# yhwu/rsicnv

Measured on AMD Instinct MI355X. Metric: bases/sec through RSI pipeline (bin+GC+NB+segment), higher is better.
Workload: dtype int32

## Files before the change

### include/rsi_hot.h

```cpp
#ifndef RSI_HOT_H
#define RSI_HOT_H
#include <stdint.h>
#ifdef __cplusplus
extern "C" {
#endif

typedef enum rsi_status {
  RSI_OK = 0,
  RSI_ERR_NO_DEVICE = -1,
  RSI_ERR_BAD_ARG = -2,
  RSI_ERR_HIP = -3,
  RSI_ERR_TOO_SMALL = -4,
  RSI_ERR_UNSUPPORTED = -5,
  RSI_ERR_INTERNAL = -6
} rsi_status;

typedef struct rsi_params {
  int32_t m;
  int32_t gcadjust;
  int32_t trans;
  int32_t merge;
  int32_t maxchkbp;
  int32_t debug;
  double cap;
// ... 165 lines not shown

int rsi_result_ncalls(const rsi_result* r, int which);
const rsi_call* rsi_result_calls(const rsi_result* r, int which);
const rsi_chrom_stats* rsi_result_stats(const rsi_result* r);
int rsi_result_noncode(const rsi_result* r, int32_t* pairs, int cap);
int rsi_result_format_row(const rsi_result* r, int i, const char* chrom, char* buf, int cap);
void rsi_result_free(rsi_result* r);

int64_t rsi_hot_fetch_i32(rsi_ctx* ctx, const char* name, int32_t* out, int64_t cap);
int64_t rsi_hot_fetch_f32(rsi_ctx* ctx, const char* name, float* out, int64_t cap);
int64_t rsi_hot_fetch_i64(rsi_ctx* ctx, const char* name, int64_t* out, int64_t cap);

int rsi_hot_debug_level_sums(rsi_ctx* ctx, const float* T, const int32_t* status, int64_t nb, int Lmax, float* sums, int32_t* counts);
int rsi_hot_debug_scan(rsi_ctx* ctx, const float* T, const int32_t* medint, int64_t nb, double RDmedian, double tmedian, double tlamda,
                       int Lmax, int32_t* status, int32_t* info);
int rsi_hot_debug_grid_median(rsi_ctx* ctx, const float* x, const int32_t* mask, int64_t nb, int mode, double center, double* out,
                              int32_t* info);
int rsi_hot_debug_grid_mad_i32(rsi_ctx* ctx, const int32_t* x, int64_t nb, double center, double* out, int32_t* info);

int rsi_hot_debug_classify(rsi_ctx* ctx, const uint8_t* fasta, int64_t n, const int64_t* start, const int64_t* end, int count,
                           uint64_t* gcbits, uint64_t* nbits);

int rsi_hot_debug_per_base(rsi_ctx* ctx, const rsi_params* p, const int32_t* depth, const uint8_t* fasta, int64_t n, const int64_t* start,
                           const int64_t* end, int count, rsi_chrom_stats* out);

int rsi_hot_kernel_times(const rsi_ctx* ctx, const char** names, float* ms, int cap);
int rsi_hot_phase_times(const rsi_ctx* ctx, const char** names, double* ms, int cap);
void rsi_hot_set_timing(rsi_ctx* ctx, int on);
void rsi_hot_set_timing_kernel(rsi_ctx* ctx, const char* name);

// ... 44 lines not shown
```

### rsicnv_amd/api.py

```python
import contextlib
import ctypes as C
import os

import numpy as np

POOL_HW_QUEUES, MIN_HW_QUEUES = 32, 4


def _queue_count(s):
    return int(s) if s is not None and 1 <= len(s) <= 9 and all(c in "0123456789" for c in s) else -1


def _process_setup(env=os.environ):
    user = env.get("RSI_HOT_HW_QUEUES")
    if user != "keep":
        want = _queue_count(user)
        if want >= 0:
            env["GPU_MAX_HW_QUEUES"] = str(min(POOL_HW_QUEUES, max(MIN_HW_QUEUES, want)))
        elif _queue_count(env.get("GPU_MAX_HW_QUEUES")) < POOL_HW_QUEUES:
            env["GPU_MAX_HW_QUEUES"] = str(POOL_HW_QUEUES)
    return max(0, _queue_count(env.get("GPU_MAX_HW_QUEUES")))


HW_QUEUES = _process_setup()

_HERE = os.path.dirname(os.path.abspath(__file__))
LIB_PATH = os.environ.get("RSI_HOT_LIB") or os.path.join(_HERE, "librsi_hot.so")

RSI_OK = 0
STATUS_NAMES = {0: "RSI_OK", -1: "RSI_ERR_NO_DEVICE", -2: "RSI_ERR_BAD_ARG", -3: "RSI_ERR_HIP",
                -4: "RSI_ERR_TOO_SMALL", -5: "RSI_ERR_UNSUPPORTED", -6: "RSI_ERR_INTERNAL"}

EXPORTS = ["rsi_default_params", "rsi_hot_create", "rsi_hot_destroy", "rsi_hot_last_error", "rsi_hot_run",
           "rsi_hot_run_device", "rsi_hot_load_depth_text", "rsi_hot_run_text", "rsi_hot_load_depth_bam", "rsi_hot_run_bam", "rsi_bam_references", "rsi_result_annotate_bam", "rsi_result_summary", "rsi_summary_format_row", "rsi_summary_format_rows", "rsi_result_pairs", "rsi_result_ncalls", "rsi_result_calls", "rsi_result_stats", "rsi_result_noncode",
           "rsi_result_format_row", "rsi_result_free", "rsi_hot_fetch_i32", "rsi_hot_fetch_f32", "rsi_hot_fetch_i64",
           "rsi_hot_kernel_times", "rsi_hot_phase_times", "rsi_hot_set_timing", "rsi_hot_process_setup", "rsi_pool_create", "rsi_pool_destroy", "rsi_pool_workers", "rsi_pool_hw_queues", "rsi_pool_worker",
           "rsi_pool_set_timing", "rsi_pool_set_timing_kernel", "rsi_hot_set_timing_kernel", "rsi_pool_set_schedule", "rsi_pool_last_error", "rsi_pool_run", "rsi_pool_run_host", "rsi_pool_submit", "rsi_pool_wait", "rsi_plot_expand", "rsi_plot_write_files", "rsi_result_log_line", "rsi_hot_debug_level_sums", "rsi_hot_debug_scan", "rsi_hot_debug_grid_median", "rsi_hot_debug_grid_mad_i32", "rsi_synth_generate_host", "rsi_synth_generate_device", "rsi_synth_write_depth_text", "rsi_synth_write_fasta", "rsi_synth_append_genome_text",
           "rsi_genome_text_open", "rsi_genome_text_next", "rsi_genome_text_release", "rsi_genome_text_copy_depth",
           "rsi_genome_text_kernel_ms", "rsi_genome_text_close", "rsi_genome_text_last_error", "rsi_hot_run_depth_device",
           "rsi_hot_last_inflate_stats", "rsi_hot_inflate_bgzf", "rsi_genome_text_inflate_stats",
           "rsi_synth_append_genome_bgzf", "rsi_genome_text_open_samples", "rsi_genome_text_samples", "rsi_genome_text_max_resident",
           "rsi_genome_text_sample_depth", "rsi_genome_text_copy_sample_depth", "rsi_synth_append_genome_samples",
           "rsi_genome_bedgraph_open", "rsi_synth_append_genome_bedgraph", "rsi_genome_bedgraph_open_indexed", "rsi_genome_text_index_range",
           "rsi_hot_set_exclude", "rsi_exclude_read_bed", "rsi_hot_debug_classify", "rsi_hot_debug_per_base",
           "rsi_hot_write_track", "rsi_hot_write_track_device", "rsi_hot_debug_track",
           "rsi_hot_write_bin_track", "rsi_hot_debug_bin_track",
           "rsi_hot_set_track_format", "rsi_hot_last_deflate_stats", "rsi_bgzf_write_eof", "rsi_hot_debug_deflate",
           "rsi_track_index_create", "rsi_track_index_free", "rsi_hot_set_track_index", "rsi_track_index_append",
           "rsi_track_index_write_tbi", "rsi_track_index_counts", "rsi_track_index_debug_tbi"]


class RsiParams(C.Structure):
# ... 401 lines not shown
        self._check(self.lib.rsi_hot_debug_level_sums(self.ctx, t.ctypes.data, s.ctypes.data, t.size, int(Lmax), sums.ctypes.data, counts.ctypes.data))
        return sums, counts

    def debug_scan(self, T, medint, RDmedian, tmedian, tlamda, Lmax):
        t = np.ascontiguousarray(T, dtype=np.float32)
        mi = np.ascontiguousarray(medint, dtype=np.int32)
        assert t.size == mi.size
        st = np.zeros(t.size, dtype=np.int32)
        info = np.zeros(4, dtype=np.int32)
        self.lib.rsi_hot_debug_scan.argtypes = [C.c_void_p, C.c_void_p, C.c_void_p, C.c_int64, C.c_double, C.c_double, C.c_double, C.c_int,
                                                C.c_void_p, C.c_void_p]
        self._check(self.lib.rsi_hot_debug_scan(self.ctx, t.ctypes.data, mi.ctypes.data, t.size, float(RDmedian), float(tmedian), float(tlamda),
                                                int(Lmax), st.ctypes.data, info.ctypes.data))
        return st, info

    GRID_MODES = {"pair": 0, "mad": 1, "host": 2}

    def debug_grid_median(self, x, mask=None, mode="pair", center=0.0):
        out = np.zeros(4, dtype=np.float64)
        info = np.zeros(8, dtype=np.int32)
        if mode == "med":
            assert mask is None
            xi = np.ascontiguousarray(x, dtype=np.int32)
            self.lib.rsi_hot_debug_grid_mad_i32.argtypes = [C.c_void_p, C.c_void_p, C.c_int64, C.c_double, C.c_void_p, C.c_void_p]
            self._check(self.lib.rsi_hot_debug_grid_mad_i32(self.ctx, xi.ctypes.data, xi.size, float(center), out.ctypes.data, info.ctypes.data))
            return out, info
        xf = np.ascontiguousarray(x, dtype=np.float32)
        mk = None if mask is None else np.ascontiguousarray(mask, dtype=np.int32)
        assert mk is None or mk.size == xf.size
        self.lib.rsi_hot_debug_grid_median.argtypes = [C.c_void_p, C.c_void_p, C.c_void_p, C.c_int64, C.c_int, C.c_double, C.c_void_p, C.c_void_p]
# ... 506 lines not shown
```

### rsicnv_amd/csrc/hostmath.h

```cpp
#pragma once
#include <math.h>
#include <stddef.h>
#include <stdint.h>
#include <algorithm>
#include <vector>

namespace rsih {

struct Quantiles { double lqt, med, uqt; };

template <class T>
inline double grid_step(const T*) { return 0.01; }
template <>
inline double grid_step<int>(const int*) { return 1.0; }

void bucket_indices_f32(const float* x, size_t n, double lo, double dy, uint32_t* idx);

template <class T>
Quantiles grid_quantiles(const T* x, size_t n) {
  const double dy = grid_step(x);
  double lo = x[0], hi = x[0], acc = 0;
  for (size_t i = 0; i < n; ++i) {
    acc += x[i];
    if (x[i] < lo) lo = x[i];
// ... 98 lines not shown
  }
  return med;
}

template <class T>
double variance_pop(const T* y, size_t n) {
  double s1 = 0.0, s2 = 0.0;
  for (size_t i = 0; i < n; ++i) { s1 += (double)y[i]; s2 += (double)y[i] * (double)y[i]; }
  const double mu = s1 / double(n);
  return s2 / double(n) - mu * mu;
}

double normal_cdf(double x);

template <class Pred>
double last_true(Pred pred) {
  if (!pred(0.0)) return -1.0;
  union { double d; uint64_t u; } lo, hi, mid;
  lo.d = 0.0; hi.d = INFINITY;
  if (pred(hi.d)) return INFINITY;
  while (hi.u - lo.u > 1) {
    mid.u = lo.u + (hi.u - lo.u) / 2;
    if (pred(mid.d)) lo = mid; else hi = mid;
  }
  return lo.d;
}
template <class Pred>
double first_true(Pred pred) {
  if (pred(0.0)) return 0.0;
  union { double d; uint64_t u; } lo, hi, mid;
  lo.d = 0.0; hi.d = INFINITY;
  if (!pred(hi.d)) return INFINITY;
  while (hi.u - lo.u > 1) {
    mid.u = lo.u + (hi.u - lo.u) / 2;
    if (pred(mid.d)) hi = mid; else lo = mid;
  }
  return hi.d;
}

}
```

### rsicnv_amd/csrc/kernels.h

```cpp
#pragma once
#include <hip/hip_runtime.h>
#include <stdint.h>
#include <mutex>
#include "device_util.h"

namespace rsik {

inline void note_launch() {
  const hipError_t e = hipGetLastError();
  if (e != hipSuccess && tl_launch_error == hipSuccess) tl_launch_error = e;
}
inline void drain_stale_errors() { (void)hipGetLastError(); tl_launch_error = hipSuccess; }
inline hipError_t take_launch_error() { const hipError_t e = tl_launch_error; tl_launch_error = hipSuccess; return e; }
#define RSI_LAUNCH(...) do { hipLaunchKernelGGL(__VA_ARGS__); rsik::note_launch(); } while (0)

constexpr int kGcLevels = 202;
constexpr int kHistValues = 65536;
constexpr int kResClasses = 32;
constexpr int kTileBases = 4096;

void launch_fasta_classify(const uint8_t* fasta, int64_t n, uint64_t* gcbits, uint64_t* nbits, int64_t nwords,
                           const FillList& fill, hipStream_t stream);
void launch_fill(const FillList& fill, hipStream_t stream);
void launch_exclude_mask(const int64_t* starts, const int64_t* ends, int count, int64_t first_start, int64_t last_end,
// ... 143 lines not shown

struct ScanParams {
  int64_t nb;
  int32_t Lmax;
  int16_t pad;
  int16_t kcap;
  double tmedian;
  double lim_del;
  double lim_dup;
};
constexpr int kMaxScanL = 10400;
constexpr int kScanLdsL = 3800;
constexpr int kScanPad = 8;
constexpr int kThrInline = 232;
struct ScanThr { double del[kThrInline]; double dup[kThrInline]; };
void launch_rsi_scan(const float* T, const int32_t* medint, const ScanParams& sp, const double* thr_del,
                     const double* thr_dup, const ScanThr* inl, uint32_t* first_del, uint32_t* first_dup, uint32_t* counters,
                     uint32_t* tiles, void* tile_ws , hipStream_t stream);
size_t scan_tile_workspace_bytes(int Lmax);
constexpr int kMaxLevels = 10416;
inline int scan_level_stride(int Lmax) { return (Lmax + 1 + kScanPad + 3) & ~3; }
constexpr int kScanRecEscapes = 0, kScanRecInexact = 1, kScanRecStop = 2 , kScanRecTiles = 8, kScanRecLevels = 16;
constexpr size_t kScanWorkBytes = 64 + 2 * (size_t)kMaxLevels * 4;
void launch_level_stop(const uint32_t* first_del, const uint32_t* first_dup, int64_t nb, int32_t Lmax, uint32_t* work, void* both,
                       unsigned int* counter, void* host_copy, size_t host_bytes, hipStream_t stream);
void launch_resolve_runs(const uint32_t* first_del, const uint32_t* first_dup, const uint32_t* levels, int64_t nb, int32_t* status,
                         int32_t* copy, uint64_t* runs, uint32_t* count, uint32_t cap, unsigned int* counter, void* host_copy,
                         uint32_t host_entries, hipStream_t stream);

struct BestSeg { double score; int32_t start; int32_t len; };
struct SegItem { int32_t run; int32_t len; int32_t Lbeg; int32_t Lend; };
constexpr int kRunsInline = 200, kItemsInline = 150;
struct RunsInline { int32_t se[2 * kRunsInline]; int32_t off[kRunsInline]; };
// ... 181 lines not shown
```

### rsicnv_amd/csrc/kernels_bin.hip

```cpp
#include <type_traits>
#include "kernels.h"
#include "device_util.h"

namespace rsik {

namespace {

constexpr int kThreads = 256;
constexpr int kMaxGrid = 256 * 2;

__device__ inline int lane_id() { return threadIdx.x & 63; }
inline int grid_for(int64_t items, int per_block) {
  int64_t g = (items + per_block - 1) / per_block;
  if (g < 1) g = 1;
  if (g > kMaxGrid) g = kMaxGrid;
  return (int)g;
}

__device__ inline uint32_t f32_key(float f) {
  const uint32_t b = __float_as_uint(f);
  return (b & 0x80000000u) ? ~b : (b | 0x80000000u);
}

__global__ __launch_bounds__(kThreads) void k_nb_raw(const int64_t* __restrict__ binsum, int64_t nb, int m,
// ... 680 lines not shown
          else cand |= __builtin_amdgcn_ballot_w64(fs <= th[u].x) | __builtin_amdgcn_ballot_w64(fs >= th[u].y);
        }
      }
    }
  };
  if (lo <= 0 || lo + count >= nb) sweep(std::true_type{}); else sweep(std::false_type{});
  if (cand != 0 && lane == 0) tiles[atomicAdd(&counters[8], 1u)] = (uint32_t)tile;
}

template <bool INL, bool GTILE, bool WIDE>
__global__ __launch_bounds__(kThreads) void k_rsi_scan(const float* __restrict__ T, const int32_t* __restrict__ medint,
                                                       ScanParams sp, const double* __restrict__ thr_del_mem,
                                                       const double* __restrict__ thr_dup_mem,
                                                       uint32_t* __restrict__ first_del, uint32_t* __restrict__ first_dup,
                                                       uint32_t* __restrict__ counters, const uint32_t* __restrict__ tiles, int parts,
                                                       ScanThr inl, unsigned char* __restrict__ gws, unsigned long long gbytes) {
  extern __shared__ __align__(16) double sm[];
  const double* __restrict__ thr_del = INL ? inl.del : thr_del_mem;
  const double* __restrict__ thr_dup = INL ? inl.dup : thr_dup_mem;
  const int Lmax = sp.Lmax, kcap = sp.kcap;
  const int halo = Lmax / 2 + 1;
  const int count = kScanTile + 2 * halo;
  auto tile_sync = [&]() { if (GTILE) drain(); __syncthreads(); };
  static_assert(GTILE || !WIDE, "a tile with 32-bit indices lives in device memory");
  using IX = typename std::conditional<WIDE, uint32_t, uint16_t>::type;
  using SL = ScanLdsT<IX>;
  SL S;
  double* const gtile = GTILE ? reinterpret_cast<double*>(gws + (size_t)blockIdx.x * gbytes) : nullptr;
  if (GTILE) scan_lds_carve(S, gtile, count, kcap); else scan_lds_carve(S, sm, count, kcap);
  __shared__ int s_c[4][kThreads];
  __shared__ double s_asum[kThreads / 64];
  __shared__ uint32_t s_amin[kThreads / 64];
  __shared__ unsigned int s_task, s_owned;
  const int fl_del = (int)floor(sp.lim_del), ce_dup = (int)ceil(sp.lim_dup);
  const double tmed = sp.tmedian;
  const int groups = (Lmax + kScanPad - 1) / kScanPad, per_part = (groups + parts - 1) / parts;
  const unsigned int ntiles = tiles ? counters[8] : (unsigned int)((sp.nb + kScanTile - 1) / kScanTile);
  const unsigned int ntasks = ntiles * (unsigned int)parts;
  for (;;) {
    tile_sync();
    if (threadIdx.x == 0) s_task = atomicAdd(&counters[9], 1u);
    tile_sync();
    const unsigned int task = s_task;
    if (task >= ntasks) break;
    const unsigned int tslot = task / (unsigned int)parts;
    const int part = (int)(task - tslot * (unsigned int)parts);
    const int Lbeg = 1 + part * per_part * kScanPad;
    int Lfin = (part + 1) * per_part * kScanPad;
    Lfin = Lfin > Lmax ? Lmax : Lfin;
    if (Lbeg > Lfin) continue;
    const int64_t tile_start = (int64_t)(tiles ? tiles[tslot] : tslot) * kScanTile;
    const int64_t lo = tile_start - halo;
// ... 432 lines not shown
  sh.gtile = Lmax > kScanLdsL;
  sh.wide = Lmax > kScanNarrowL;
  if (!sh.gtile) while (sh.kcap > 0 && scan_lds_bytes(sh.count, sh.kcap) + 4 * kThreads * sizeof(int) + 1024 > 160 * 1024) --sh.kcap;
  sh.tile_bytes = scan_lds_bytes(sh.count, sh.kcap, sh.wide ? 4 : 2);
  sh.grid = kGTileGrid;
  if (sh.gtile) {
    const size_t slice = (sh.tile_bytes + 255) & ~size_t(255);
    if (slice * (size_t)sh.grid > kGTileBudget) sh.grid = (int)std::max<size_t>(1, kGTileBudget / slice);
  }
  return sh;
}
size_t scan_tile_workspace_bytes(int Lmax) {
  const ScanShape sh = scan_tile_shape(Lmax);
  return sh.gtile ? (size_t)sh.grid * ((sh.tile_bytes + 255) & ~size_t(255)) : 0;
}
void launch_rsi_scan(const float* T, const int32_t* medint, const ScanParams& sp_in, const double* thr_del, const double* thr_dup,
                     const ScanThr* inl, uint32_t* first_del, uint32_t* first_dup, uint32_t* counters, uint32_t* tiles, void* tile_ws,
                     hipStream_t stream) {
  ScanParams sp = sp_in;
  const ScanShape sh = scan_tile_shape(sp.Lmax);
  const bool gtile = sh.gtile;
  sp.kcap = (int16_t)sh.kcap;
  const size_t tile_bytes = sh.tile_bytes;
  const size_t lds = gtile ? 0 : tile_bytes;
  const unsigned long long gbytes = (tile_bytes + 255) & ~size_t(255);
  const int64_t ntiles = (sp.nb + kScanTile - 1) / kScanTile;
  static const ScanThr none{};
  const char* det_env = getenv("RSI_HOT_SCAN_DETECT");
  const size_t dlds = detect_lds_bytes(sp.Lmax);
  const bool detect = tiles != nullptr && !(det_env && atoi(det_env) == 0) && dlds + kThreads * 8 + 64 <= 160 * 1024;
  int parts = 1;
  if (detect || gtile) {
    const int groups = (sp.Lmax + kScanPad - 1) / kScanPad;
    parts = groups < kScanPartsMax ? groups : kScanPartsMax;
    if (const char* pe = getenv("RSI_HOT_SCAN_PARTS")) { const int v = atoi(pe); if (v >= 1 && v <= groups) parts = v; }
  }
  if (detect) {
    const int dgrid = (int)((sp.nb + kDetBins - 1) / kDetBins);
    if (inl) { RSI_ALLOW_FULL_LDS(k_scan_detect<true>); RSI_LAUNCH(k_scan_detect<true>, dim3(dgrid), dim3(kThreads), dlds, stream, T, sp.nb, sp.Lmax, nullptr, nullptr, tiles, counters, *inl); }
    else { RSI_ALLOW_FULL_LDS(k_scan_detect<false>); RSI_LAUNCH(k_scan_detect<false>, dim3(dgrid), dim3(kThreads), dlds, stream, T, sp.nb, sp.Lmax, thr_del, thr_dup, tiles, counters, none); }
  }
  int64_t grid = ntiles * parts;
  const int64_t resident = gtile ? sh.grid : 256 * (int64_t)(lds > 80 * 1024 ? 1 : lds > 52 * 1024 ? 2 : lds > 39 * 1024 ? 3 : 4);
  if ((detect || gtile) && grid > resident) grid = resident;
  const uint32_t* list = detect ? tiles : nullptr;
  unsigned char* gws = static_cast<unsigned char*>(tile_ws);
#define RSI_SCAN(INL_, GT_, WIDE_, ...) do { RSI_ALLOW_FULL_LDS((k_rsi_scan<INL_, GT_, WIDE_>));                                             \
    RSI_LAUNCH((k_rsi_scan<INL_, GT_, WIDE_>), dim3((unsigned)grid), dim3(kThreads), lds, stream, T, medint, sp, __VA_ARGS__, first_del, first_dup, \
               counters, list, parts, inl ? *inl : none, gws, gbytes); } while (0)
  if (gtile && sh.wide) RSI_SCAN(false, true, true, thr_del, thr_dup);
  else if (gtile) { if (inl) RSI_SCAN(true, true, false, nullptr, nullptr); else RSI_SCAN(false, true, false, thr_del, thr_dup); }
  else { if (inl) RSI_SCAN(true, false, false, nullptr, nullptr); else RSI_SCAN(false, false, false, thr_del, thr_dup); }
#undef RSI_SCAN
}
void launch_level_stop(const uint32_t* first_del, const uint32_t* first_dup, int64_t nb, int32_t Lmax, uint32_t* work, void* both,
                       unsigned int* counter, void* host_copy, size_t host_bytes, hipStream_t stream) {
  const size_t lds = (size_t)(Lmax + 1) * 8;
  if (lds + 256 <= 160 * 1024) {
    RSI_ALLOW_FULL_LDS(k_level_stop<false>);
    RSI_LAUNCH(k_level_stop<false>, dim3(grid_for(nb, kThreads * 16)), dim3(kThreads), lds, stream, first_del, first_dup, nb,
                       Lmax, work, static_cast<uint2*>(both), counter, host_copy, (unsigned int)host_bytes);
  } else {
    RSI_LAUNCH(k_level_stop<true>, dim3(grid_for(nb, kThreads * 16)), dim3(kThreads), 0, stream, first_del, first_dup, nb,
                       Lmax, work, static_cast<uint2*>(both), counter, host_copy, (unsigned int)host_bytes);
// ... 32 lines not shown
```

### rsicnv_amd/csrc/pipeline.hip

```cpp
#include <new>
#include "pipeline_internal.h"
#include "pipeline_steps.h"

using namespace rsik;
using namespace rsip;
using rsih::Candidate;
using rsih::Region;

namespace {

struct ScanOut {
  double tmedian1 = 0, tsigma1 = 0, tlamda1 = 0, tmedian2 = 0, tsigma2 = 0, tlamda2 = 0;
  int Lmax = 0;
  rsih::IntSpan status2;
  std::vector<int> run_status;
  std::vector<rsih::IntSpan::Range> run_ranges;
  std::vector<Candidate> segs;
  uint32_t escapes = 0, inexact = 0;
  uint32_t tiles_listed = 0;
  std::vector<uint32_t> level_log[4];
  uint32_t stop_levels[4] = {0, 0, 0, 0};
  std::vector<std::string> fs_lines;
};

// ... 85 lines not shown
  ex.src[0] = d_g; ex.dst[0] = slot->g; ex.bytes[0] = 2 * sizeof(GridMedian);
  ex.src[1] = small + kOffRawMin; ex.dst[1] = &slot->rawmin_inv; ex.bytes[1] = 4;
  FillList fl{};
  if (fill_pass >= 0) scan_fill_list(ctx, fill_pass, nb, fl);
  { Timer t(ctx, "hist_walk"); launch_hist_walk(d_x, d_mask, nb, 1, center, d_center, gc, d_g + 1, &ex, &fl, ctx->stream); }
  *out = slot;
  return RSI_OK;
}
struct Selection { const float* d_x; const int32_t* d_mask; int64_t nb; int use_abs; double center; };
int grid_result(rsi_ctx* ctx, const GridMedian& g, const Selection& sel, double* med, uint64_t* count) {
  if (g.flags & kGridEmpty) { *count = 0; *med = 0; return RSI_OK; }
  if (g.flags & kGridNonFinite) return fail(ctx, RSI_ERR_UNSUPPORTED, "non-finite value in the transformed bins");
  if (g.flags & kGridDegenerate) return selection_mean(ctx, sel.d_x, sel.d_mask, sel.nb, sel.use_abs, sel.center, med, count);
  *med = g.med; *count = g.count;
  return RSI_OK;
}

void scan_thresholds(double tmedian, double tlamda, int Lmax, std::vector<double>& del, std::vector<double>& dup) {
  del.assign((size_t)Lmax + 1 + kScanPad, -INFINITY);
  dup.assign((size_t)Lmax + 1 + kScanPad, INFINITY);
  del[0] = -1.0;
  for (int L = 1; L <= Lmax; ++L) {
    const double dL = (double)L, sq = sqrt(dL);
    auto score = [&](double sum) { const float meanf = (float)(sum / dL); return ((double)meanf - tmedian) * sq; };
    del[L] = rsih::last_true([&](double s) { return !(score(s) > -tlamda); });
    dup[L] = rsih::first_true([&](double s) { return !(score(s) < tlamda); });
  }
}

constexpr uint32_t kEagerBounds = 1024;
int runs_from_export(rsi_ctx* ctx, const uint32_t* slot, const uint64_t* d_list, std::vector<Region>& runs) {
  const uint32_t cnt = slot[0];
  runs.clear();
  if (cnt == 0) return RSI_OK;
  if (cnt > kMaxRunEntries) return fail(ctx, RSI_ERR_UNSUPPORTED, "boundary list overflow");
  std::vector<uint64_t> raw(cnt);
  memcpy(raw.data(), slot + 2, (size_t)std::min(cnt, kEagerBounds) * 8);
  if (cnt > kEagerBounds) {
    HIPCHK(copy_d2h(ctx, raw.data() + kEagerBounds, d_list + kEagerBounds, (size_t)(cnt - kEagerBounds) * 8));
    HIPCHK(CTX_SYNC());
  }
  if (!rsih::boundary_pairs(raw.data(), raw.size(), false, runs)) return fail(ctx, RSI_ERR_INTERNAL, "unbalanced run boundaries");
// ... 200 lines not shown
    set_global_error(ctx->err);
    failed = true;
    return false;
  }
  bool wait() {
    const double t0 = now_ms();
    const bool r = ok(ctx_sync(ctx));
    kernel_wait_ms += now_ms() - t0;
    ++launches;
    return r;
  }
 public:
  bool failed = false;
};

int scan_pass(rsi_ctx* ctx, int pass, const float* d_T, const int32_t* d_medint, int64_t nb, double RDmedian, double tmedian,
              double tlamda, int Lmax, int32_t* d_status, int32_t* d_copy, const uint32_t** work_slot, const uint32_t** runs_slot,
              std::vector<uint32_t>* spill) {
  uint8_t* small = ctx->small.as<uint8_t>();
  std::vector<double> del, dup;
  scan_thresholds(tmedian, tlamda, Lmax, del, dup);
  const size_t nthr = (size_t)Lmax + 1 + kScanPad;
  ScanThr inl;
  const bool use_inl = nthr <= (size_t)kThrInline;
  double* d_del = nullptr;
  double* d_dup = nullptr;
  if (use_inl) {
    for (size_t k = 0; k < (size_t)kThrInline; ++k) { inl.del[k] = k < nthr ? del[k] : -INFINITY; inl.dup[k] = k < nthr ? dup[k] : INFINITY; }
  } else {
    HIPCHK(ctx->thr.ensure(nthr * 16));
    d_del = ctx->thr.as<double>();
    d_dup = d_del + nthr;
    del.insert(del.end(), dup.begin(), dup.end());
    HIPCHK(copy_h2d(ctx, d_del, del.data(), 2 * nthr * 8));
  }
  uint32_t* work = reinterpret_cast<uint32_t*>(small + kOffScanPass + (size_t)pass * kScanPassBytes);
  if (Lmax > kMaxL) {
    const size_t dev_bytes = (64 + 2 * (size_t)scan_level_stride(Lmax) * 4 + 255) & ~size_t(255);
    HIPCHK(ctx->scan_work_big.ensure(2 * dev_bytes));
    work = reinterpret_cast<uint32_t*>(ctx->scan_work_big.as<uint8_t>() + (size_t)pass * dev_bytes);
    HIPCHK(hipMemsetAsync(work, 0, dev_bytes, ctx->stream));
    if (pass == 0) ctx->phases.push_back({"scan.long (Lmax > 10400)", 1.0});
  }
  uint32_t* d_first_del = ctx->first_del.as<uint32_t>();
  uint32_t* d_first_dup = d_first_del + ((nb + 3) & ~int64_t(3));
  unsigned int* d_done = reinterpret_cast<unsigned int*>(small + kOffDone) + kDoneBinSlot;
  uint32_t* d_count = reinterpret_cast<uint32_t*>(small + kOffCounters) + 4;
  const size_t work_bytes = 64 + ((size_t)scan_level_stride(Lmax) + (size_t)Lmax + 1) * 4;
  if (scan_tile_workspace_bytes(Lmax)) HIPCHK(ctx->scan_ws.ensure(scan_tile_workspace_bytes(Lmax)));
  uint32_t* rslot = static_cast<uint32_t*>(mb_alloc(ctx, 8 + (size_t)kEagerBounds * 8));
  uint32_t* wslot = static_cast<uint32_t*>(work_bytes <= kMailboxBytes / 8 ? mb_alloc(ctx, work_bytes) : nullptr);
  const bool spilled = !wslot && Lmax > kMaxL && spill;
  if (spilled) spill->assign((work_bytes + 3) / 4, 0u);
  if ((!wslot && !spilled) || !rslot) return fail(ctx, RSI_ERR_INTERNAL, "out of pinned mailbox memory");
  ScanParams sp;
  sp.nb = nb; sp.Lmax = Lmax; sp.pad = 0; sp.tmedian = tmedian;
  sp.lim_del = RDmedian * 0.75; sp.lim_dup = RDmedian * 1.25;
  { Timer t(ctx, "rsi_scan"); launch_rsi_scan(d_T, d_medint, sp, d_del, d_dup, use_inl ? &inl : nullptr, d_first_del, d_first_dup, work, ctx->scan_tiles.as<uint32_t>(), ctx->scan_ws.p, ctx->stream); }
  { Timer t(ctx, "level_stop"); launch_level_stop(d_first_del, d_first_dup, nb, Lmax, work, ctx->runs.p, d_done + 2, wslot, wslot ? work_bytes : 0, ctx->stream); }
  if (spilled) { HIPCHK(hipMemcpyAsync(spill->data(), work, work_bytes, hipMemcpyDeviceToHost, ctx->stream)); wslot = spill->data(); }
  { Timer t(ctx, "resolve_runs"); launch_resolve_runs(d_first_del, d_first_dup, work + 2, nb, d_status, d_copy, ctx->runs.as<uint64_t>(), d_count, kMaxRunEntries, d_done + 3, rslot, kEagerBounds, ctx->stream); }
  *work_slot = wslot; *runs_slot = rslot;
  return RSI_OK;
}

int run_scan(rsi_ctx* ctx, const rsi_params& P, bool use_med, const float* d_T, int64_t nb, double RDmedian,
             double factor, int LmaxBase, ChainOut* first, double nb_med_raw, double nb_del_raw, double nb_dup_raw, ScanOut& out) {
  const int32_t* d_medint = ctx->binmed.as<int32_t>();
  double tmedian, absmed;
  uint64_t cnt;
  int rc;
  rsih::NbScaled lv{0, 0};
  {
// ... 33 lines not shown
    const rsih::ScanRecord rec{w, Lmax};
    if (clipped && !rec.sweeps_stopped(nb)) return fail(ctx, RSI_ERR_TOO_SMALL, "fewer bins than the scan length, and a sweep reached them all (the reference exits in runmean)");
    out.escapes += rec.escapes(); out.inexact = rec.inexact(); out.tiles_listed += rec.tiles_listed();
    for (int k = 0; k < 2; ++k) {
      out.level_log[2 * pass + k].assign(rec.level_counts(k), rec.level_counts(k) + Lmax + 1);
      out.stop_levels[2 * pass + k] = rec.stop_level(k);
    }
    return RSI_OK;
  };

  int32_t* d_st1 = ctx->status1.as<int32_t>();
  int32_t* d_st1f = ctx->status1f.as<int32_t>();
  int32_t* d_st2 = ctx->status2.as<int32_t>();
  const uint32_t* wslot = nullptr;
  const uint32_t* rslot = nullptr;
  { Phase ph(ctx, "scan.pass"); GateShared gs(ctx); if ((rc = scan_pass(ctx, 0, d_T, d_medint, nb, RDmedian, tmedian, tlamda, Lmax, d_st1, d_st1f, &wslot, &rslot, &spill1)) != RSI_OK) return rc; }

  Phase ph_filter(ctx, "scan.filterstatus");
  const int nlev = 2 * Lmax + 1;
  uint32_t* fs_slot = long_scan ? nullptr : static_cast<uint32_t*>(mb_alloc(ctx, (size_t)nlev * 8));
  if (!fs_slot && !long_scan) return fail(ctx, RSI_ERR_INTERNAL, "out of pinned mailbox memory");
  if (!long_scan) {
    GateShared gs(ctx);
    Timer t(ctx, "level_sums");
    launch_level_sums(d_T, d_st1, nb, Lmax, ctx->fs_ws.p, kMaxL, kFsListCap, ctx->fs_out.as<float>(),
                      reinterpret_cast<unsigned int*>(ctx->small.as<uint8_t>() + kOffDone) + kDoneBinSlot + 4, fs_slot, ctx->stream);
  }
  { Phase phc(ctx, "fs.wait"); HIPCHK(CTX_SYNC()); }
  if ((rc = take_record(wslot, 0)) != RSI_OK) return rc;
  {
    Phase phs(ctx, "fs.sums");
// ... 41 lines not shown
  const GridMedian* g2 = second->g;
  {
    GateShared gs_q2(ctx);
    const bool wide2 = (g2[0].flags & kGridTooWide) != 0;
    if ((rc = wide2 ? grid_median(ctx, d_T, d_st1f, nb, 0, 0.0, &tmed2, &k) : grid_result(ctx, g2[0], Selection{d_T, d_st1f, nb, 0, 0.0}, &tmed2, &k)) != RSI_OK) return rc;
    if (k > (uint64_t)(nb / 2)) {
      tmedian = tmed2;
      if ((rc = (wide2 || (g2[1].flags & (kGridTooWide)) || (g2[0].flags & kGridDegenerate)) ? grid_median(ctx, d_T, d_st1f, nb, 1, tmedian, &absmed, &cnt)
                                                        : grid_result(ctx, g2[1], Selection{d_T, d_st1f, nb, 1, tmedian}, &absmed, &cnt)) != RSI_OK) return rc;
      const rsih::Lamda l2 = rsih::lamda_from_mad(absmed, factor, target);
      tsigma = l2.tsigma; tlamda = l2.tlamda;
    }
  }
  out.tmedian2 = tmedian; out.tsigma2 = tsigma; out.tlamda2 = tlamda;
  ph_q2.stop();
  { Phase ph(ctx, "scan.pass"); GateShared gs(ctx); if ((rc = scan_pass(ctx, 1, d_T, d_medint, nb, RDmedian, tmedian, tlamda, Lmax, d_st2, nullptr, &wslot, &rslot, &spill2)) != RSI_OK) return rc; }
  Phase ph_seg(ctx, "scan.segments");
  GateShared gs_seg(ctx);

  HIPCHK(CTX_SYNC());
  std::vector<Region> runs;
  if ((rc = runs_from_export(ctx, rslot, ctx->runs.as<uint64_t>(), runs)) != RSI_OK) return rc;
  if ((rc = take_record(wslot, 1)) != RSI_OK) return rc;
  out.status2 = rsih::IntSpan();
  out.segs.clear();
  if (runs.empty()) return RSI_OK;
  std::vector<int64_t> poff;
  std::vector<SegItem> items;
  int64_t pairs_per_item = 1 << 16;
  if (!ctx->gate || ctx->gate->lonely()) {
    int64_t total = 0;
// ... 1064 lines not shown
    launch_fill(fl, ctx->stream);
  }
  const uint32_t* wslot = nullptr;
  const uint32_t* rslot = nullptr;
  std::vector<uint32_t> spill;
  const int rc = scan_pass(ctx, 0, ctx->tnb.as<float>(), ctx->binmed.as<int32_t>(), nb, RDmedian, tmedian, tlamda, Lmax, ctx->status1.as<int32_t>(),
                           ctx->status1f.as<int32_t>(), &wslot, &rslot, &spill);
  if (rc != RSI_OK) return rc;
  HIPCHK(hipMemcpyAsync(status, ctx->status1.p, (size_t)nb * 4, hipMemcpyDeviceToHost, ctx->stream));
  HIPCHK(CTX_SYNC());
  const rsih::ScanRecord rec{wslot, Lmax};
  if (info) { info[0] = (int32_t)rec.tiles_listed(); info[1] = (int32_t)rec.escapes(); info[2] = (int32_t)rec.inexact(); info[3] = 0; }
  return RSI_OK;
}

int rsi_hot_debug_grid_median(rsi_ctx* ctx, const float* x, const int32_t* mask, int64_t nb, int mode, double center, double* out,
                              int32_t* info) {
  int rc;
  if (!x || mode < 0 || mode > 2) return fail(ctx, RSI_ERR_BAD_ARG, "bad argument");
  if ((rc = grid_debug_enter(ctx, nb, out, info)) != RSI_OK) return rc;
  HIPCHK(ctx->tnb.ensure((size_t)nb * 4));
  HIPCHK(hipMemcpyAsync(ctx->tnb.p, x, (size_t)nb * 4, hipMemcpyHostToDevice, ctx->stream));
  ctx->have_nb = false;
  const int32_t* d_mask = nullptr;
  if (mask) {
    HIPCHK(ctx->status1f.ensure((size_t)nb * 4));
    HIPCHK(hipMemcpyAsync(ctx->status1f.p, mask, (size_t)nb * 4, hipMemcpyHostToDevice, ctx->stream));
    d_mask = ctx->status1f.as<int32_t>();
  }
  const float* d_x = ctx->tnb.as<float>();
// ... 167 lines not shown
```

### rsicnv_amd/csrc/pipeline_steps.h

```cpp
#pragma once
#include <math.h>
#include <stdio.h>
#include <string.h>
#include <algorithm>
#include <string>
#include <vector>
#include "host_calls.h"
#include "hostmath.h"
#include "kernels.h"

namespace rsih {

inline bool boundary_pairs(const uint64_t* raw, size_t cnt, bool end_exclusive, std::vector<Region>& out) {
  out.clear();
  std::vector<int64_t> s, e;
  for (size_t i = 0; i < cnt; ++i) { const uint64_t v = raw[i]; ((v & 1) ? e : s).push_back((int64_t)(v >> 1)); }
  if (s.size() != e.size()) return false;
  std::sort(s.begin(), s.end());
  std::sort(e.begin(), e.end());
  for (size_t i = 0; i < s.size(); ++i) out.push_back({(int)s[i], (int)(e[i] - (end_exclusive ? 1 : 0))});
  return true;
}

inline float unkey_f32(uint32_t k) {
// ... 126 lines not shown
  } else {
    s.target = tmedian * sqrt(2.0);
    const Lamda l = lamda_from_mad(absmed, factor, s.target);
    s.tsigma = l.tsigma; s.tlamda = l.tlamda;
    if (threshold > 0) s.tlamda = tmedian * threshold;
    const double q = s.tlamda * 4 / (tmedian + 0.001);
    s.cal_max = (int)(q * q);
    s.dev = tmedian * 0.6;
  }
  s.Lmax = LmaxBase;
  if (s.Lmax < s.cal_max) s.Lmax = s.cal_max;
  s.Lmax_ref = s.Lmax;
  s.clipped = s.Lmax > nb;
  if (s.clipped) s.Lmax = (int)nb;
  return s;
}

struct ScanRecord {
  const uint32_t* w;
  int Lmax;
  uint32_t escapes() const { return w[rsik::kScanRecEscapes]; }
  uint32_t inexact() const { return w[rsik::kScanRecInexact]; }
  uint32_t stop_level(int sweep) const { return w[rsik::kScanRecStop + sweep]; }
  uint32_t tiles_listed() const { return w[rsik::kScanRecTiles]; }
  const uint32_t* level_counts(int sweep) const { return w + rsik::kScanRecLevels + (size_t)sweep * rsik::scan_level_stride(Lmax); }
  bool sweeps_stopped(int64_t nb) const {
    for (int k = 0; k < 2; ++k) {
      const uint32_t* cnt = level_counts(k);
      uint64_t cum = 0;
      for (uint32_t L = 0; L <= stop_level(k) && L <= (uint32_t)Lmax; ++L) cum += cnt[L];
// ... 86 lines not shown
```

Before: 257.6 billion.

## Reuse first-pass scan tile detection list for second pass via guard thresholds

The first scan pass now runs its tile-detection kernel with widened guard thresholds that cover a band of plausible second-pass medians and lambdas. If the second pass's thresholds fall inside that guard, it skips its own detection launch and reuses the first pass's tile list and counters. Threshold bisection also gets a seed near the analytic solution to cut host-side search iterations. The cost is a conservative (larger) tile list in pass one and extra guard threshold computation and transfer.

```diff
diff --git a/include/rsi_hot.h b/include/rsi_hot.h
--- a/include/rsi_hot.h
+++ b/include/rsi_hot.h
@@ -203,6 +203,9 @@
 int rsi_hot_debug_level_sums(rsi_ctx* ctx, const float* T, const int32_t* status, int64_t nb, int Lmax, float* sums, int32_t* counts);
 int rsi_hot_debug_scan(rsi_ctx* ctx, const float* T, const int32_t* medint, int64_t nb, double RDmedian, double tmedian, double tlamda,
                        int Lmax, int32_t* status, int32_t* info);
+int rsi_hot_debug_scan_pair(rsi_ctx* ctx, const float* T, const int32_t* medint, int64_t nb, double RDmedian, double tmedian1,
+                            double tlamda1, double target, double tmedian2, double tlamda2, int Lmax, int32_t* status1, int32_t* status2,
+                            int32_t* info);
 int rsi_hot_debug_grid_median(rsi_ctx* ctx, const float* x, const int32_t* mask, int64_t nb, int mode, double center, double* out,
                               int32_t* info);
 int rsi_hot_debug_grid_mad_i32(rsi_ctx* ctx, const int32_t* x, int64_t nb, double center, double* out, int32_t* info);
diff --git a/rsicnv_amd/api.py b/rsicnv_amd/api.py
--- a/rsicnv_amd/api.py
+++ b/rsicnv_amd/api.py
@@ -35,7 +35,7 @@
            "rsi_hot_run_device", "rsi_hot_load_depth_text", "rsi_hot_run_text", "rsi_hot_load_depth_bam", "rsi_hot_run_bam", "rsi_bam_references", "rsi_result_annotate_bam", "rsi_result_summary", "rsi_summary_format_row", "rsi_summary_format_rows", "rsi_result_pairs", "rsi_result_ncalls", "rsi_result_calls", "rsi_result_stats", "rsi_result_noncode",
            "rsi_result_format_row", "rsi_result_free", "rsi_hot_fetch_i32", "rsi_hot_fetch_f32", "rsi_hot_fetch_i64",
            "rsi_hot_kernel_times", "rsi_hot_phase_times", "rsi_hot_set_timing", "rsi_hot_process_setup", "rsi_pool_create", "rsi_pool_destroy", "rsi_pool_workers", "rsi_pool_hw_queues", "rsi_pool_worker",
-           "rsi_pool_set_timing", "rsi_pool_set_timing_kernel", "rsi_hot_set_timing_kernel", "rsi_pool_set_schedule", "rsi_pool_last_error", "rsi_pool_run", "rsi_pool_run_host", "rsi_pool_submit", "rsi_pool_wait", "rsi_plot_expand", "rsi_plot_write_files", "rsi_result_log_line", "rsi_hot_debug_level_sums", "rsi_hot_debug_scan", "rsi_hot_debug_grid_median", "rsi_hot_debug_grid_mad_i32", "rsi_synth_generate_host", "rsi_synth_generate_device", "rsi_synth_write_depth_text", "rsi_synth_write_fasta", "rsi_synth_append_genome_text",
+           "rsi_pool_set_timing", "rsi_pool_set_timing_kernel", "rsi_hot_set_timing_kernel", "rsi_pool_set_schedule", "rsi_pool_last_error", "rsi_pool_run", "rsi_pool_run_host", "rsi_pool_submit", "rsi_pool_wait", "rsi_plot_expand", "rsi_plot_write_files", "rsi_result_log_line", "rsi_hot_debug_level_sums", "rsi_hot_debug_scan", "rsi_hot_debug_scan_pair", "rsi_hot_debug_grid_median", "rsi_hot_debug_grid_mad_i32", "rsi_synth_generate_host", "rsi_synth_generate_device", "rsi_synth_write_depth_text", "rsi_synth_write_fasta", "rsi_synth_append_genome_text",
            "rsi_genome_text_open", "rsi_genome_text_next", "rsi_genome_text_release", "rsi_genome_text_copy_depth",
            "rsi_genome_text_kernel_ms", "rsi_genome_text_close", "rsi_genome_text_last_error", "rsi_hot_run_depth_device",
            "rsi_hot_last_inflate_stats", "rsi_hot_inflate_bgzf", "rsi_genome_text_inflate_stats",
@@ -467,6 +467,19 @@
                                                 int(Lmax), st.ctypes.data, info.ctypes.data))
         return st, info
 
+    def debug_scan_pair(self, T, medint, RDmedian, tmedian1, tlamda1, target, tmedian2, tlamda2, Lmax):
+        t = np.ascontiguousarray(T, dtype=np.float32)
+        mi = np.ascontiguousarray(medint, dtype=np.int32)
+        assert t.size == mi.size
+        st1 = np.zeros(t.size, dtype=np.int32)
+        st2 = np.zeros(t.size, dtype=np.int32)
+        info = np.zeros(8, dtype=np.int32)
+        self.lib.rsi_hot_debug_scan_pair.argtypes = [C.c_void_p, C.c_void_p, C.c_void_p, C.c_int64] + [C.c_double] * 6 + [C.c_int] + [C.c_void_p] * 3
+        self._check(self.lib.rsi_hot_debug_scan_pair(self.ctx, t.ctypes.data, mi.ctypes.data, t.size, float(RDmedian), float(tmedian1), float(tlamda1),
+                                                     float(target), float(tmedian2), float(tlamda2), int(Lmax), st1.ctypes.data, st2.ctypes.data,
+                                                     info.ctypes.data))
+        return st1, st2, info
+
     GRID_MODES = {"pair": 0, "mad": 1, "host": 2}
 
     def debug_grid_median(self, x, mask=None, mode="pair", center=0.0):
diff --git a/rsicnv_amd/csrc/hostmath.h b/rsicnv_amd/csrc/hostmath.h
--- a/rsicnv_amd/csrc/hostmath.h
+++ b/rsicnv_amd/csrc/hostmath.h
@@ -136,11 +136,14 @@
 double normal_cdf(double x);
 
 template <class Pred>
-double last_true(Pred pred) {
-  if (!pred(0.0)) return -1.0;
+double last_true(Pred pred, double near = 0.0) {
   union { double d; uint64_t u; } lo, hi, mid;
-  lo.d = 0.0; hi.d = INFINITY;
-  if (pred(hi.d)) return INFINITY;
+  lo.d = near * (1.0 - 9.5367431640625e-07); hi.d = near * (1.0 + 9.5367431640625e-07);
+  if (!(near > 0.0 && hi.d < INFINITY && lo.d < hi.d && pred(lo.d) && !pred(hi.d))) {
+    if (!pred(0.0)) return -1.0;
+    lo.d = 0.0; hi.d = INFINITY;
+    if (pred(hi.d)) return INFINITY;
+  }
   while (hi.u - lo.u > 1) {
     mid.u = lo.u + (hi.u - lo.u) / 2;
     if (pred(mid.d)) lo = mid; else hi = mid;
@@ -148,11 +151,14 @@
   return lo.d;
 }
 template <class Pred>
-double first_true(Pred pred) {
-  if (pred(0.0)) return 0.0;
+double first_true(Pred pred, double near = 0.0) {
   union { double d; uint64_t u; } lo, hi, mid;
-  lo.d = 0.0; hi.d = INFINITY;
-  if (!pred(hi.d)) return INFINITY;
+  lo.d = near * (1.0 - 9.5367431640625e-07); hi.d = near * (1.0 + 9.5367431640625e-07);
+  if (!(near > 0.0 && hi.d < INFINITY && lo.d < hi.d && !pred(lo.d) && pred(hi.d))) {
+    if (pred(0.0)) return 0.0;
+    lo.d = 0.0; hi.d = INFINITY;
+    if (!pred(hi.d)) return INFINITY;
+  }
   while (hi.u - lo.u > 1) {
     mid.u = lo.u + (hi.u - lo.u) / 2;
     if (pred(mid.d)) hi = mid; else lo = mid;
diff --git a/rsicnv_amd/csrc/kernels.h b/rsicnv_amd/csrc/kernels.h
--- a/rsicnv_amd/csrc/kernels.h
+++ b/rsicnv_amd/csrc/kernels.h
@@ -181,9 +181,12 @@
 constexpr int kScanPad = 8;
 constexpr int kThrInline = 232;
 struct ScanThr { double del[kThrInline]; double dup[kThrInline]; };
+struct ScanListing { const ScanThr* det_inl = nullptr; const double* det_del = nullptr; const double* det_dup = nullptr; const uint32_t* list_from = nullptr; };
 void launch_rsi_scan(const float* T, const int32_t* medint, const ScanParams& sp, const double* thr_del,
                      const double* thr_dup, const ScanThr* inl, uint32_t* first_del, uint32_t* first_dup, uint32_t* counters,
-                     uint32_t* tiles, void* tile_ws , hipStream_t stream);
+                     uint32_t* tiles, void* tile_ws , hipStream_t stream,
+                     const ScanListing* how = nullptr);
+bool scan_detects(int Lmax);
 size_t scan_tile_workspace_bytes(int Lmax);
 constexpr int kMaxLevels = 10416;
 inline int scan_level_stride(int Lmax) { return (Lmax + 1 + kScanPad + 3) & ~3; }
diff --git a/rsicnv_amd/csrc/kernels_bin.hip b/rsicnv_amd/csrc/kernels_bin.hip
--- a/rsicnv_amd/csrc/kernels_bin.hip
+++ b/rsicnv_amd/csrc/kernels_bin.hip
@@ -718,7 +718,8 @@
                                                        const double* __restrict__ thr_dup_mem,
                                                        uint32_t* __restrict__ first_del, uint32_t* __restrict__ first_dup,
                                                        uint32_t* __restrict__ counters, const uint32_t* __restrict__ tiles, int parts,
-                                                       ScanThr inl, unsigned char* __restrict__ gws, unsigned long long gbytes) {
+                                                       ScanThr inl, unsigned char* __restrict__ gws, unsigned long long gbytes,
+                                                       const uint32_t* list_ctr ) {
   extern __shared__ __align__(16) double sm[];
   const double* __restrict__ thr_del = INL ? inl.del : thr_del_mem;
   const double* __restrict__ thr_dup = INL ? inl.dup : thr_dup_mem;
@@ -739,7 +740,8 @@
   const int fl_del = (int)floor(sp.lim_del), ce_dup = (int)ceil(sp.lim_dup);
   const double tmed = sp.tmedian;
   const int groups = (Lmax + kScanPad - 1) / kScanPad, per_part = (groups + parts - 1) / parts;
-  const unsigned int ntiles = tiles ? counters[8] : (unsigned int)((sp.nb + kScanTile - 1) / kScanTile);
+  const unsigned int ntiles = tiles ? list_ctr[8] : (unsigned int)((sp.nb + kScanTile - 1) / kScanTile);
+  if (tiles && list_ctr != counters && blockIdx.x == 0 && threadIdx.x == 0) { counters[1] = list_ctr[1]; counters[8] = ntiles; }
   const unsigned int ntasks = ntiles * (unsigned int)parts;
   for (;;) {
     tile_sync();
@@ -1202,9 +1204,13 @@
   const ScanShape sh = scan_tile_shape(Lmax);
   return sh.gtile ? (size_t)sh.grid * ((sh.tile_bytes + 255) & ~size_t(255)) : 0;
 }
+bool scan_detects(int Lmax) {
+  const char* det_env = getenv("RSI_HOT_SCAN_DETECT");
+  return !(det_env && atoi(det_env) == 0) && detect_lds_bytes(Lmax) + kThreads * 8 + 64 <= 160 * 1024;
+}
 void launch_rsi_scan(const float* T, const int32_t* medint, const ScanParams& sp_in, const double* thr_del, const double* thr_dup,
                      const ScanThr* inl, uint32_t* first_del, uint32_t* first_dup, uint32_t* counters, uint32_t* tiles, void* tile_ws,
-                     hipStream_t stream) {
+                     hipStream_t stream, const ScanListing* how) {
   ScanParams sp = sp_in;
   const ScanShape sh = scan_tile_shape(sp.Lmax);
   const bool gtile = sh.gtile;
@@ -1214,19 +1220,23 @@
   const unsigned long long gbytes = (tile_bytes + 255) & ~size_t(255);
   const int64_t ntiles = (sp.nb + kScanTile - 1) / kScanTile;
   static const ScanThr none{};
-  const char* det_env = getenv("RSI_HOT_SCAN_DETECT");
   const size_t dlds = detect_lds_bytes(sp.Lmax);
-  const bool detect = tiles != nullptr && !(det_env && atoi(det_env) == 0) && dlds + kThreads * 8 + 64 <= 160 * 1024;
+  const bool detect = tiles != nullptr && scan_detects(sp.Lmax);
+  const uint32_t* list_ctr = detect && how && how->list_from ? how->list_from : counters;
   int parts = 1;
   if (detect || gtile) {
     const int groups = (sp.Lmax + kScanPad - 1) / kScanPad;
     parts = groups < kScanPartsMax ? groups : kScanPartsMax;
     if (const char* pe = getenv("RSI_HOT_SCAN_PARTS")) { const int v = atoi(pe); if (v >= 1 && v <= groups) parts = v; }
   }
-  if (detect) {
+  if (detect && list_ctr == counters) {
     const int dgrid = (int)((sp.nb + kDetBins - 1) / kDetBins);
-    if (inl) { RSI_ALLOW_FULL_LDS(k_scan_detect<true>); RSI_LAUNCH(k_scan_detect<true>, dim3(dgrid), dim3(kThreads), dlds, stream, T, sp.nb, sp.Lmax, nullptr, nullptr, tiles, counters, *inl); }
-    else { RSI_ALLOW_FULL_LDS(k_scan_detect<false>); RSI_LAUNCH(k_scan_detect<false>, dim3(dgrid), dim3(kThreads), dlds, stream, T, sp.nb, sp.Lmax, thr_del, thr_dup, tiles, counters, none); }
+    const bool own = how && (how->det_inl || how->det_del);
+    const ScanThr* dinl = own ? how->det_inl : inl;
+    const double* ddel = own ? how->det_del : thr_del;
+    const double* ddup = own ? how->det_dup : thr_dup;
+    if (dinl) { RSI_ALLOW_FULL_LDS(k_scan_detect<true>); RSI_LAUNCH(k_scan_detect<true>, dim3(dgrid), dim3(kThreads), dlds, stream, T, sp.nb, sp.Lmax, nullptr, nullptr, tiles, counters, *dinl); }
+    else { RSI_ALLOW_FULL_LDS(k_scan_detect<false>); RSI_LAUNCH(k_scan_detect<false>, dim3(dgrid), dim3(kThreads), dlds, stream, T, sp.nb, sp.Lmax, ddel, ddup, tiles, counters, none); }
   }
   int64_t grid = ntiles * parts;
   const int64_t resident = gtile ? sh.grid : 256 * (int64_t)(lds > 80 * 1024 ? 1 : lds > 52 * 1024 ? 2 : lds > 39 * 1024 ? 3 : 4);
@@ -1235,7 +1245,7 @@
   unsigned char* gws = static_cast<unsigned char*>(tile_ws);
 #define RSI_SCAN(INL_, GT_, WIDE_, ...) do { RSI_ALLOW_FULL_LDS((k_rsi_scan<INL_, GT_, WIDE_>));                                             \
     RSI_LAUNCH((k_rsi_scan<INL_, GT_, WIDE_>), dim3((unsigned)grid), dim3(kThreads), lds, stream, T, medint, sp, __VA_ARGS__, first_del, first_dup, \
-               counters, list, parts, inl ? *inl : none, gws, gbytes); } while (0)
+               counters, list, parts, inl ? *inl : none, gws, gbytes, list_ctr); } while (0)
   if (gtile && sh.wide) RSI_SCAN(false, true, true, thr_del, thr_dup);
   else if (gtile) { if (inl) RSI_SCAN(true, true, false, nullptr, nullptr); else RSI_SCAN(false, true, false, thr_del, thr_dup); }
   else { if (inl) RSI_SCAN(true, false, false, nullptr, nullptr); else RSI_SCAN(false, false, false, thr_del, thr_dup); }
diff --git a/rsicnv_amd/csrc/pipeline.hip b/rsicnv_amd/csrc/pipeline.hip
--- a/rsicnv_amd/csrc/pipeline.hip
+++ b/rsicnv_amd/csrc/pipeline.hip
@@ -123,18 +123,6 @@
   if (g.flags & kGridDegenerate) return selection_mean(ctx, sel.d_x, sel.d_mask, sel.nb, sel.use_abs, sel.center, med, count);
   *med = g.med; *count = g.count;
   return RSI_OK;
-}
-
-void scan_thresholds(double tmedian, double tlamda, int Lmax, std::vector<double>& del, std::vector<double>& dup) {
-  del.assign((size_t)Lmax + 1 + kScanPad, -INFINITY);
-  dup.assign((size_t)Lmax + 1 + kScanPad, INFINITY);
-  del[0] = -1.0;
-  for (int L = 1; L <= Lmax; ++L) {
-    const double dL = (double)L, sq = sqrt(dL);
-    auto score = [&](double sum) { const float meanf = (float)(sum / dL); return ((double)meanf - tmedian) * sq; };
-    del[L] = rsih::last_true([&](double s) { return !(score(s) > -tlamda); });
-    dup[L] = rsih::first_true([&](double s) { return !(score(s) < tlamda); });
-  }
 }
 
 constexpr uint32_t kEagerBounds = 1024;
@@ -365,25 +353,51 @@
   bool failed = false;
 };
 
+struct ScanShare {
+  double target = 0;
+  bool guarded = false;
+  rsih::ScanGuard guard;
+  const uint32_t* list_work = nullptr;
+  bool detected[2] = {false, false};
+};
+bool scan_reuse_enabled() { const char* e = getenv("RSI_HOT_SCAN_REUSE"); return !(e && atoi(e) == 0); }
 int scan_pass(rsi_ctx* ctx, int pass, const float* d_T, const int32_t* d_medint, int64_t nb, double RDmedian, double tmedian,
               double tlamda, int Lmax, int32_t* d_status, int32_t* d_copy, const uint32_t** work_slot, const uint32_t** runs_slot,
-              std::vector<uint32_t>* spill) {
+              std::vector<uint32_t>* spill, ScanShare* share = nullptr) {
   uint8_t* small = ctx->small.as<uint8_t>();
   std::vector<double> del, dup;
-  scan_thresholds(tmedian, tlamda, Lmax, del, dup);
+  rsih::scan_thresholds(tmedian, tlamda, Lmax, del, dup);
   const size_t nthr = (size_t)Lmax + 1 + kScanPad;
-  ScanThr inl;
+  const bool detects = scan_detects(Lmax);
+  ScanListing how;
+  if (share && pass == 0 && detects && Lmax <= kMaxL && scan_reuse_enabled()) {
+    share->guard = rsih::scan_guard_thresholds(tmedian, tlamda, share->target, Lmax, del, dup);
+    share->guarded = true;
+  }
+  const bool reuse = share && pass == 1 && share->guarded && detects && rsih::scan_guard_covers(share->guard.del, share->guard.dup, del, dup, Lmax);
+  const bool guard_now = share && pass == 0 && share->guarded;
+  ScanThr inl, ginl;
   const bool use_inl = nthr <= (size_t)kThrInline;
   double* d_del = nullptr;
   double* d_dup = nullptr;
   if (use_inl) {
     for (size_t k = 0; k < (size_t)kThrInline; ++k) { inl.del[k] = k < nthr ? del[k] : -INFINITY; inl.dup[k] = k < nthr ? dup[k] : INFINITY; }
+    if (guard_now) {
+      const rsih::ScanGuard& g = share->guard;
+      for (size_t k = 0; k < (size_t)kThrInline; ++k) { ginl.del[k] = k < nthr ? g.del[k] : -INFINITY; ginl.dup[k] = k < nthr ? g.dup[k] : INFINITY; }
+      how.det_inl = &ginl;
+    }
   } else {
-    HIPCHK(ctx->thr.ensure(nthr * 16));
+    HIPCHK(ctx->thr.ensure(nthr * 32));
     d_del = ctx->thr.as<double>();
     d_dup = d_del + nthr;
     del.insert(del.end(), dup.begin(), dup.end());
-    HIPCHK(copy_h2d(ctx, d_del, del.data(), 2 * nthr * 8));
+    if (guard_now) {
+      del.insert(del.end(), share->guard.del.begin(), share->guard.del.end());
+      del.insert(del.end(), share->guard.dup.begin(), share->guard.dup.end());
+      how.det_del = d_del + 2 * nthr; how.det_dup = d_del + 3 * nthr;
+    }
+    HIPCHK(copy_h2d(ctx, d_del, del.data(), del.size() * 8));
   }
   uint32_t* work = reinterpret_cast<uint32_t*>(small + kOffScanPass + (size_t)pass * kScanPassBytes);
   if (Lmax > kMaxL) {
@@ -407,7 +421,13 @@
   ScanParams sp;
   sp.nb = nb; sp.Lmax = Lmax; sp.pad = 0; sp.tmedian = tmedian;
   sp.lim_del = RDmedian * 0.75; sp.lim_dup = RDmedian * 1.25;
-  { Timer t(ctx, "rsi_scan"); launch_rsi_scan(d_T, d_medint, sp, d_del, d_dup, use_inl ? &inl : nullptr, d_first_del, d_first_dup, work, ctx->scan_tiles.as<uint32_t>(), ctx->scan_ws.p, ctx->stream); }
+  if (reuse) how.list_from = share->list_work;
+  if (guard_now) share->list_work = work;
+  if (share) {
+    share->detected[pass] = detects && !reuse;
+    if (pass == 1 && detects) ctx->phases.push_back({reuse ? "scan.pass2 list reused" : "scan.pass2 detection", 1.0});
+  }
+  { Timer t(ctx, "rsi_scan"); launch_rsi_scan(d_T, d_medint, sp, d_del, d_dup, use_inl ? &inl : nullptr, d_first_del, d_first_dup, work, ctx->scan_tiles.as<uint32_t>(), ctx->scan_ws.p, ctx->stream, &how); }
   { Timer t(ctx, "level_stop"); launch_level_stop(d_first_del, d_first_dup, nb, Lmax, work, ctx->runs.p, d_done + 2, wslot, wslot ? work_bytes : 0, ctx->stream); }
   if (spilled) { HIPCHK(hipMemcpyAsync(spill->data(), work, work_bytes, hipMemcpyDeviceToHost, ctx->stream)); wslot = spill->data(); }
   { Timer t(ctx, "resolve_runs"); launch_resolve_runs(d_first_del, d_first_dup, work + 2, nb, d_status, d_copy, ctx->runs.as<uint64_t>(), d_count, kMaxRunEntries, d_done + 3, rslot, kEagerBounds, ctx->stream); }
@@ -471,7 +491,9 @@
   int32_t* d_st2 = ctx->status2.as<int32_t>();
   const uint32_t* wslot = nullptr;
   const uint32_t* rslot = nullptr;
-  { Phase ph(ctx, "scan.pass"); GateShared gs(ctx); if ((rc = scan_pass(ctx, 0, d_T, d_medint, nb, RDmedian, tmedian, tlamda, Lmax, d_st1, d_st1f, &wslot, &rslot, &spill1)) != RSI_OK) return rc; }
+  ScanShare share;
+  share.target = target;
+  { Phase ph(ctx, "scan.pass"); GateShared gs(ctx); if ((rc = scan_pass(ctx, 0, d_T, d_medint, nb, RDmedian, tmedian, tlamda, Lmax, d_st1, d_st1f, &wslot, &rslot, &spill1, &share)) != RSI_OK) return rc; }
 
   Phase ph_filter(ctx, "scan.filterstatus");
   const int nlev = 2 * Lmax + 1;
@@ -543,7 +565,7 @@
   }
   out.tmedian2 = tmedian; out.tsigma2 = tsigma; out.tlamda2 = tlamda;
   ph_q2.stop();
-  { Phase ph(ctx, "scan.pass"); GateShared gs(ctx); if ((rc = scan_pass(ctx, 1, d_T, d_medint, nb, RDmedian, tmedian, tlamda, Lmax, d_st2, nullptr, &wslot, &rslot, &spill2)) != RSI_OK) return rc; }
+  { Phase ph(ctx, "scan.pass"); GateShared gs(ctx); if ((rc = scan_pass(ctx, 1, d_T, d_medint, nb, RDmedian, tmedian, tlamda, Lmax, d_st2, nullptr, &wslot, &rslot, &spill2, &share)) != RSI_OK) return rc; }
   Phase ph_seg(ctx, "scan.segments");
   GateShared gs_seg(ctx);
 
@@ -1638,6 +1660,54 @@
   return RSI_OK;
 }
 
+int rsi_hot_debug_scan_pair(rsi_ctx* ctx, const float* T, const int32_t* medint, int64_t nb, double RDmedian, double tmedian1,
+                            double tlamda1, double target, double tmedian2, double tlamda2, int Lmax, int32_t* status1, int32_t* status2,
+                            int32_t* info ) {
+  if (!ctx || !T || !medint || !status1 || !status2 || !info || nb <= 0 || nb >= (1ll << 31) - 4096 || Lmax < 1 || Lmax > kHardMaxL || Lmax > nb)
+    return fail(ctx, RSI_ERR_BAD_ARG, "bad argument");
+  HIPCHK(hipSetDevice(ctx->device));
+  if (!ctx_enter(ctx)) return RSI_ERR_HIP;
+  mailbox_reset(ctx);
+  ctx->nb = nb; ctx->run_m = 0;
+  HIPCHK(ctx->small.ensure(kSmallBytes));
+  HIPCHK(ctx->tnb.ensure((size_t)nb * 4));
+  HIPCHK(ctx->binmed.ensure((size_t)nb * 4));
+  HIPCHK(ctx->first_del.ensure((size_t)(2 * nb + 8) * 4));
+  HIPCHK(ctx->status1.ensure((size_t)nb * 4));
+  HIPCHK(ctx->status1f.ensure((size_t)nb * 4));
+  HIPCHK(ctx->status2.ensure((size_t)nb * 4));
+  HIPCHK(ctx->runs.ensure((size_t)kMaxRunEntries * 8));
+  HIPCHK(ctx->scan_tiles.ensure((size_t)(nb / 256 + 2) * 4));
+  HIPCHK(hipMemcpyAsync(ctx->tnb.p, T, (size_t)nb * 4, hipMemcpyHostToDevice, ctx->stream));
+  HIPCHK(hipMemcpyAsync(ctx->binmed.p, medint, (size_t)nb * 4, hipMemcpyHostToDevice, ctx->stream));
+  HIPCHK(hipMemsetAsync(ctx->small.p, 0, kHeaderBytes, ctx->stream));
+  ScanShare share;
+  share.target = target;
+  const uint32_t* wslot[2] = {nullptr, nullptr};
+  const uint32_t* rslot = nullptr;
+  std::vector<uint32_t> spill[2];
+  for (int pass = 0; pass < 2; ++pass) {
+    FillList fl{};
+    void* keep = ctx->fs_ws.p;
+    ctx->fs_ws.p = nullptr;
+    scan_fill_list(ctx, pass, nb, fl);
+    ctx->fs_ws.p = keep;
+    launch_fill(fl, ctx->stream);
+    const int rc = scan_pass(ctx, pass, ctx->tnb.as<float>(), ctx->binmed.as<int32_t>(), nb, RDmedian, pass ? tmedian2 : tmedian1, pass ? tlamda2 : tlamda1,
+                             Lmax, (pass ? ctx->status2 : ctx->status1).as<int32_t>(), pass ? nullptr : ctx->status1f.as<int32_t>(), &wslot[pass],
+                             &rslot, &spill[pass], &share);
+    if (rc != RSI_OK) return rc;
+    HIPCHK(hipMemcpyAsync(pass ? status2 : status1, (pass ? ctx->status2 : ctx->status1).p, (size_t)nb * 4, hipMemcpyDeviceToHost, ctx->stream));
+  }
+  HIPCHK(CTX_SYNC());
+  for (int pass = 0; pass < 2; ++pass) {
+    const rsih::ScanRecord rec{wslot[pass], Lmax};
+    info[4 * pass] = (int32_t)rec.tiles_listed(); info[4 * pass + 1] = (int32_t)rec.escapes(); info[4 * pass + 2] = (int32_t)rec.inexact();
+    info[4 * pass + 3] = share.detected[pass] ? 1 : 0;
+  }
+  return RSI_OK;
+}
+
 int rsi_hot_debug_grid_median(rsi_ctx* ctx, const float* x, const int32_t* mask, int64_t nb, int mode, double center, double* out,
                               int32_t* info) {
   int rc;
diff --git a/rsicnv_amd/csrc/pipeline_steps.h b/rsicnv_amd/csrc/pipeline_steps.h
--- a/rsicnv_amd/csrc/pipeline_steps.h
+++ b/rsicnv_amd/csrc/pipeline_steps.h
@@ -164,6 +164,41 @@
   s.clipped = s.Lmax > nb;
   if (s.clipped) s.Lmax = (int)nb;
   return s;
+}
+
+inline void scan_thresholds(double tmedian, double tlamda, int Lmax, std::vector<double>* del, std::vector<double>* dup) {
+  if (del) { del->assign((size_t)Lmax + 1 + rsik::kScanPad, -INFINITY); (*del)[0] = -1.0; }
+  if (dup) dup->assign((size_t)Lmax + 1 + rsik::kScanPad, INFINITY);
+  for (int L = 1; L <= Lmax; ++L) {
+    const double dL = (double)L, sq = sqrt(dL);
+    auto score = [&](double sum) { const float meanf = (float)(sum / dL); return ((double)meanf - tmedian) * sq; };
+    if (del) (*del)[(size_t)L] = last_true([&](double s) { return !(score(s) > -tlamda); }, dL * (tmedian - tlamda / sq));
+    if (dup) (*dup)[(size_t)L] = first_true([&](double s) { return !(score(s) < tlamda); }, dL * (tmedian + tlamda / sq));
+  }
+}
+inline void scan_thresholds(double tmedian, double tlamda, int Lmax, std::vector<double>& del, std::vector<double>& dup) {
+  scan_thresholds(tmedian, tlamda, Lmax, &del, &dup);
+}
+struct ScanGuard { std::vector<double> del, dup; double lamda = 0, dt = 0; };
+inline ScanGuard scan_guard_thresholds(double tmedian1, double tlamda1, double target, int Lmax, const std::vector<double>& del1,
+                                       const std::vector<double>& dup1) {
+  ScanGuard g;
+  g.lamda = std::min(tlamda1, target);
+  g.dt = 0.5 * g.lamda / sqrt((double)Lmax);
+  scan_thresholds(tmedian1 + g.dt, g.lamda, Lmax, &g.del, nullptr);
+  scan_thresholds(tmedian1 - g.dt, g.lamda, Lmax, nullptr, &g.dup);
+  for (int L = 1; L <= Lmax; ++L) {
+    g.del[(size_t)L] = std::max(g.del[(size_t)L], del1[(size_t)L]);
+    g.dup[(size_t)L] = std::min(g.dup[(size_t)L], dup1[(size_t)L]);
+  }
+  return g;
+}
+inline bool scan_guard_covers(const std::vector<double>& gdel, const std::vector<double>& gdup, const std::vector<double>& del,
+                              const std::vector<double>& dup, int Lmax) {
+  const size_t need = (size_t)Lmax + 1;
+  if (Lmax < 1 || gdel.size() < need || gdup.size() < need || del.size() < need || dup.size() < need) return false;
+  for (size_t L = 1; L < need; ++L) if (!(del[L] <= gdel[L] && dup[L] >= gdup[L])) return false;
+  return true;
 }
 
 struct ScanRecord {
```

Result: no change. 257.6 billion (-0.0%).
